# PJLab-ADG/OpenPCSeg

Measured on AMD Instinct MI355X. Metric: LiDAR frames/sec training MinkUNet-34 SemanticKITTI, higher is better.
Workload: dtype f32; 1 GPU; MinkUNet-34 cr1.0 train step, 12 x 120k-pt synthetic SemanticKITTI scans/GPU, fp32; global_batch=12, voxels_per_gpu_batch=1158864, parallelism=dp1, wgrad=fp32

## Files before the change

include/pcseg_hip.h:

```cpp
#ifndef PCSEG_HIP_H_
#define PCSEG_HIP_H_

#include <stddef.h>
#include <stdint.h>

#ifdef __cplusplus
extern "C" {
#endif

#define PCS_OK 0
#define PCS_EINVAL (-1)
#define PCS_EWORKSPACE (-2)
#define PCS_ELAUNCH (-3)
#define PCS_EUNSUPPORTED (-4)

#define PCS_ABI_VERSION 12

int pcs_abi_version(void);
const char *pcs_last_error(void);

int pcs_hash(const int32_t *coords, int64_t n, int64_t *out, void *stream);

int pcs_kernel_hash(const int32_t *coords, int64_t n, const int32_t *offsets, int32_t K,
                    int64_t *out, void *stream);
// ... 128 lines not shown
                             void *stream);
int pcs_range_sample_bwd_csr_f32(const float *gout, const int64_t *order, const int64_t *rowptr, const float *wts,
                                 int32_t B, int32_t C, int32_t H, int32_t W, float *gimg, void *stream);

int32_t pcs_bn_num_partials(void);
int pcs_bn_stats_f32(const float *x, int64_t n, int32_t c, float *partial_ws, double *sums, void *stream);
int pcs_bn_reduce_partials(const double *partial, int64_t nrows, int32_t c, int64_t n, double *sums, void *stream);
int pcs_bn_reduce_partials_finalize(const double *partial, int64_t nrows, int32_t c, int64_t n, double eps, double momentum,
                                    float *running_mean, float *running_var, double *sums, double *stat, void *stream);
int pcs_bn_finalize_f32(const double *sums, double count, const double *count_dev, int32_t c, double eps,
                        double momentum, float *running_mean, float *running_var, double *stat, void *stream);
int pcs_bn_apply_f32(const float *x, const float *res, const double *stat, const float *w, const float *b,
                     int64_t n, int32_t c, int32_t relu, float *y, uint32_t *mask, int64_t ldy, const float *tail,
                     int32_t ctail, void *stream);
int pcs_bn_bwd_stats_f32(const float *dy, const float *x, const float *y, const uint32_t *mask, const double *stat,
                         int64_t n, int32_t c, int32_t relu, float *partial_ws, double *sums2, int64_t sums2_doubles,
                         int64_t lddy, void *stream);
int pcs_bn_bwd_apply_f32(const float *dy, const float *x, const float *y, const uint32_t *mask, const double *stat,
                         const double *sums2, double count, const double *count_dev, const float *w, int64_t n,
                         int32_t c, int32_t relu, float *dx, float *dres, int64_t lddy, void *stream);
int pcs_bn_stats_h(const void *x, int64_t n, int32_t c, int32_t dtype, float *partial_ws, double *sums, void *stream);
int pcs_bn_apply_h(const void *x, const void *res, const double *stat, const float *w, const float *b, int64_t n,
                   int32_t c, int32_t relu, int32_t dtype, void *y, uint32_t *mask, int64_t ldy, const void *tail,
                   int32_t ctail, void *stream);
int pcs_bn_bwd_stats_h(const void *dy, const void *x, const void *y, const uint32_t *mask, const double *stat, int64_t n,
                       int32_t c, int32_t relu, int32_t dtype, float *partial_ws, double *sums2, int64_t sums2_doubles,
                       int64_t lddy, void *stream);
int pcs_bn_bwd_apply_h(const void *dy, const void *x, const void *y, const uint32_t *mask, const double *stat,
                       const double *sums2, double count, const double *count_dev, const float *w, int64_t n,
                       int32_t c, int32_t relu, int32_t dtype, void *dx, void *dres, int64_t lddy, void *stream);
int pcs_bn_bwd_apply_act(const void *dy, const void *x, const void *y, const uint32_t *mask, const double *stat,
                         const double *sums2, double count, const double *count_dev, const float *w, int64_t n, int32_t c,
                         int32_t relu, int32_t dtype, float in_slope, void *dx, void *dres, int64_t lddy, void *stream);

int pcs_recon_gate_f32(const float *a0, const float *a1, const float *a2, const float *x, const double *stat3,
                       const float *gamma3, const float *beta3, int64_t n, int32_t c, float *out, void *stream);
int pcs_recon_gate_h(const void *a0, const void *a1, const void *a2, const void *x, const double *stat3, const float *gamma3,
                     const float *beta3, int64_t n, int32_t c, int32_t dtype, void *out, void *stream);
int pcs_recon_gate_bwd_stats_f32(const float *dy, const float *x, const float *a0, const float *a1, const float *a2,
                                 const double *stat3, const float *gamma3, const float *beta3, int64_t n, int32_t c,
                                 float *partial_ws, double *sums2, int64_t sums2_doubles, void *stream);
int pcs_recon_gate_bwd_stats_h(const void *dy, const void *x, const void *a0, const void *a1, const void *a2,
                               const double *stat3, const float *gamma3, const float *beta3, int64_t n, int32_t c,
                               int32_t dtype, float *partial_ws, double *sums2, int64_t sums2_doubles, void *stream);
int pcs_recon_gate_bwd_apply_f32(const float *dy, const float *x, const float *a0, const float *a1, const float *a2,
                                 const double *stat3, const float *gamma3, const float *beta3, const double *sums2,
                                 double count, const double *count_dev, int64_t n, int32_t c, float *dx_gate, float *da0,
                                 float *da1, float *da2, void *stream);
int pcs_recon_gate_bwd_apply_h(const void *dy, const void *x, const void *a0, const void *a1, const void *a2,
                               const double *stat3, const float *gamma3, const float *beta3, const double *sums2, double count,
                               const double *count_dev, int64_t n, int32_t c, int32_t dtype, void *dx_gate, void *da0,
                               void *da1, void *da2, void *stream);

int pcs_quantize_floor(const void *points, int32_t is_float, int64_t n, int32_t row_stride,
                       const double *voxel_size3, int32_t *coords, int32_t *bbox, void *stream);
int pcs_quantize_keys(const int32_t *coords, int64_t n, const int32_t *bbox, int64_t *keys, void *stream);
int pcs_quantize_frame_keys(const int32_t *coords, const int64_t *frames, int64_t n, const int32_t *bbox, int64_t *keys, void *stream);
int pcs_quantize_flags(const int64_t *sorted_keys, int64_t n, int32_t *flags, void *stream);
int pcs_quantize_emit(const int32_t *flags, const int64_t *rank, const int64_t *perm, const int32_t *coords,
                      int64_t n, int32_t *vox, int64_t *index, int64_t *inverse, void *stream);

int pcs_unique_emit(const int32_t *flags, const int64_t *rank, const int64_t *perm, const int64_t *sorted_keys,
                    int64_t n, int64_t *uniq, int64_t *inverse, int64_t *rowptr, void *stream);

int pcs_conv_x3_applies(int32_t cin, int32_t cout, int32_t K);
int32_t pcs_conv_x3_column_tiles(int32_t cout);
// ... 65 lines not shown
```

openpcseg_amd/csrc/norm.hip:

```cpp
#include "row_storage.h"

using namespace pcs;

namespace {

template <int V> struct NV;
template <> struct NV<4> { using T = float4; };
template <> struct NV<1> { using T = float; };
template <int V, typename ET> __device__ __forceinline__ typename NV<V>::T ldv(ET, const void *p, int64_t e) {
  const Acc<V> a = widen(ET{}, *reinterpret_cast<const typename Raw<ET, V>::T *>(reinterpret_cast<const typename Elem<ET>::T *>(p) + e));
  if constexpr (V == 4) return make_float4(a.f[0], a.f[1], a.f[2], a.f[3]);
  else return a.f[0];
}
template <typename ET> __device__ __forceinline__ void stv(ET, void *p, int64_t e, const float4 &v) {
  *reinterpret_cast<typename Raw<ET, 4>::T *>(reinterpret_cast<typename Elem<ET>::T *>(p) + e) = narrow(ET{}, Acc<4>{{v.x, v.y, v.z, v.w}});
}
template <typename ET> __device__ __forceinline__ void stv(ET, void *p, int64_t e, const float &v) {
  reinterpret_cast<typename Elem<ET>::T *>(p)[e] = narrow(ET{}, Acc<1>{{v}});
}

__device__ __forceinline__ float comp(const float4 &v, int i) { return i == 0 ? v.x : (i == 1 ? v.y : (i == 2 ? v.z : v.w)); }
__device__ __forceinline__ float comp(const float &v, int) { return v; }
__device__ __forceinline__ void setc(float4 &v, int i, float s) { if (i == 0) v.x = s; else if (i == 1) v.y = s; else if (i == 2) v.z = s; else v.w = s; }
__device__ __forceinline__ void setc(float &v, int, float s) { v = s; }
// ... 211 lines not shown
  if (!(count > 0.0)) count = 1.0;
  for (int j = threadIdx.x; j < cv; j += blockDim.x) {
    float mean[V], invstd[V], k1[V], k2[V], ws[V];
#pragma unroll
    for (int q = 0; q < V; ++q) {
      const int ch = j * V + q;
      mean[q] = (float)stat[ch]; invstd[q] = (float)stat[c + ch];
      k1[q] = (float)(sums2[ch] / count);
      k2[q] = (float)(sums2[c + ch] / count);
      ws[q] = invstd[q] * (w ? w[ch] : 1.f);
    }
#pragma unroll 4
    for (int64_t i = (int64_t)blockIdx.x * blockDim.y + threadIdx.y; i < n; i += (int64_t)gridDim.x * blockDim.y) {
      const VT gv = ldv<V>(ET{}, dy, i * lddy + (int64_t)j * V);
      const VT xv = ldv<V>(ET{}, x, i * c + (int64_t)j * V);
      VT yv; unsigned bits = 0xFu;
      if (relu) {
        if (V == 4 && mask) bits = (mask[i * (c >> 5) + (j >> 3)] >> (4 * (j & 7))) & 0xFu;
        else yv = ldv<V>(ET{}, y, i * c + (int64_t)j * V);
      }
      VT o, r;
#pragma unroll
      for (int q = 0; q < V; ++q) {
        float g = comp(gv, q);
        if (relu && ((V == 4 && mask) ? !((bits >> q) & 1u) : comp(yv, q) <= 0.f)) g = 0.f;
        const float xh = (comp(xv, q) - mean[q]) * invstd[q];
        float d = (g - k1[q] - xh * k2[q]) * ws[q];
        if (in_slope != 1.f && !(comp(xv, q) > 0.f)) d *= in_slope;
        setc(o, q, d);
        setc(r, q, g);
      }
      stv(ET{}, dx, i * c + (int64_t)j * V, o);
      if (dres) stv(ET{}, dres, i * c + (int64_t)j * V, r);
    }
  }
}

template <int V> RowLaunch geo(int64_t n, int c) { return row_launch(n, c / V, kRowsExact4); }

}

extern "C" int32_t pcs_bn_num_partials(void) { return kStatBlocks + 1; }

static bool al_v4(int dtype, const void *p) { return aligned(p, dtype == 0 ? 16 : 8); }

static int bn_partial(bool bwd, int dtype, const void *x, const void *dy, const void *y, const uint32_t *mask, const double *stat,
                      int64_t n, int c, int relu, float *partial, double *sums, hipStream_t st, int64_t lddy = 0) {
  if (lddy == 0) lddy = c;
  if (lddy < c) { set_error("pcs_bn: row stride of dy smaller than c"); return PCS_EINVAL; }
  const bool vec = (c & 3) == 0 && (lddy & 3) == 0 && al_v4(dtype, x) && al_v4(dtype, dy) && al_v4(dtype, y);
  if (mask && (!vec || (c & 31))) { set_error("pcs_bn: the ReLU bit mask needs c % 32 == 0 and aligned rows"); return PCS_EUNSUPPORTED; }
  const int V = vec ? 4 : 1, cv = c / V;
  const dim3 block = row_launch(n, cv, kRowsExact4).block;
  const size_t lds = (size_t)block.y * 2 * block.x * V * sizeof(float);
  if (vec) {
    if (bwd) PCS_DTYPE(dtype, hipLaunchKernelGGL((bn_partial_kernel<true, 4, ET>), dim3(kStatBlocks), block, lds, st, x, dy, y, mask, stat, n, c, cv, relu, partial, lddy));
    else PCS_DTYPE(dtype, hipLaunchKernelGGL((bn_partial_kernel<false, 4, ET>), dim3(kStatBlocks), block, lds, st, x, dy, y, mask, stat, n, c, cv, relu, partial, lddy));
  } else {
    if (bwd) PCS_DTYPE(dtype, hipLaunchKernelGGL((bn_partial_kernel<true, 1, ET>), dim3(kStatBlocks), block, lds, st, x, dy, y, mask, stat, n, c, cv, relu, partial, lddy));
    else PCS_DTYPE(dtype, hipLaunchKernelGGL((bn_partial_kernel<false, 1, ET>), dim3(kStatBlocks), block, lds, st, x, dy, y, mask, stat, n, c, cv, relu, partial, lddy));
  }
  const float *pivot = bwd ? nullptr : partial + (size_t)kStatBlocks * 2 * c;
  hipLaunchKernelGGL(bn_reduce_kernel<float>, dim3((unsigned)ceil_div(c, kRedCh)), dim3(kRedCh, kRedLanes), 0, st, partial, kStatBlocks, c,
                     pivot, n, sums, bwd ? 0 : 1, bwd ? reinterpret_cast<float *>(sums + 2 * (size_t)c) : (float *)nullptr,
                     (double *)nullptr, 0.0, 0.0, (float *)nullptr, (float *)nullptr);
  return check_launch("pcs_bn_partial");
// ... 99 lines not shown
                                    double *sums2, int64_t sums2_doubles, int64_t lddy, void *stream) {
  if (n < 0 || c <= 0 || (n > 0 && (!dy || !x || (relu && !y && !mask))) || !stat || !partial_ws || !sums2) { set_error("pcs_bn_bwd_stats: bad args"); return PCS_EINVAL; }
  if (sums2_doubles < 3 * (int64_t)c) { set_error("pcs_bn_bwd_stats: sums2 must hold 3c doubles (2c sums + the same 2c values as floats)"); return PCS_EWORKSPACE; }
  return bn_partial(true, 0, x, dy, y, mask, stat, n, c, relu, partial_ws, sums2, as_stream(stream), lddy);
}
extern "C" int pcs_bn_bwd_stats_h(const void *dy, const void *x, const void *y, const uint32_t *mask,
                                  const double *stat, int64_t n, int32_t c, int32_t relu, int32_t dtype, float *partial_ws,
                                  double *sums2, int64_t sums2_doubles, int64_t lddy, void *stream) {
  if (n < 0 || c <= 0 || (n > 0 && (!dy || !x || (relu && !y && !mask))) || !stat || !partial_ws || !sums2 || !is_half(dtype)) { set_error("pcs_bn_bwd_stats_h: bad args"); return PCS_EINVAL; }
  if (sums2_doubles < 3 * (int64_t)c) { set_error("pcs_bn_bwd_stats_h: sums2 must hold 3c doubles (2c sums + the same 2c values as floats)"); return PCS_EWORKSPACE; }
  return bn_partial(true, dtype, x, dy, y, mask, stat, n, c, relu, partial_ws, sums2, as_stream(stream), lddy);
}

extern "C" int pcs_bn_bwd_apply_f32(const float *dy, const float *x, const float *y, const uint32_t *mask,
                                    const double *stat, const double *sums2, double count, const double *count_dev,
                                    const float *w, int64_t n, int32_t c, int32_t relu, float *dx, float *dres,
                                    int64_t lddy, void *stream) {
  return bn_bwd_apply_any(0, dy, x, y, mask, stat, sums2, count, count_dev, w, n, c, relu, dx, dres, lddy, stream);
}
extern "C" int pcs_bn_bwd_apply_act(const void *dy, const void *x, const void *y, const uint32_t *mask,
                                    const double *stat, const double *sums2, double count, const double *count_dev,
                                    const float *w, int64_t n, int32_t c, int32_t relu, int32_t dtype, float in_slope, void *dx,
                                    void *dres, int64_t lddy, void *stream) {
  if (dtype < 0 || dtype > 2 || !(in_slope > 0.f)) { set_error("pcs_bn_bwd_apply_act: dtype must be 0 / 1 / 2 and in_slope > 0"); return PCS_EINVAL; }
  return bn_bwd_apply_any(dtype, dy, x, y, mask, stat, sums2, count, count_dev, w, n, c, relu, dx, dres, lddy, stream, in_slope);
}
extern "C" int pcs_bn_bwd_apply_h(const void *dy, const void *x, const void *y, const uint32_t *mask,
                                  const double *stat, const double *sums2, double count, const double *count_dev,
                                  const float *w, int64_t n, int32_t c, int32_t relu, int32_t dtype, void *dx, void *dres,
                                  int64_t lddy, void *stream) {
  if (bad_half("pcs_bn_bwd_apply_h", dtype, false)) return PCS_EINVAL;
  return bn_bwd_apply_any(dtype, dy, x, y, mask, stat, sums2, count, count_dev, w, n, c, relu, dx, dres, lddy, stream);
}
```

openpcseg_amd/fused.py:

```python
import torch
import torch.distributed as dist
from torch import nn
from torch.autograd import Function

from . import native
from .sparse import SparseTensor


def _world():
    return dist.get_world_size() if dist.is_available() and dist.is_initialized() else 1


def _syncing(sync):
    if not sync or not (dist.is_available() and dist.is_initialized()):
        return False
    import os
    return dist.get_world_size() > 1 or os.environ.get("PCS_SYNC_WORLD1") == "1"


_STATS_GROUP = {}


def _stats_group():
    import os
# ... 66 lines not shown
        ctx.in_slope = in_slope
        return y

    @staticmethod
    def backward(ctx, dy):
        be = native.backend()
        x, gate, stat, weight, count_dev = ctx.saved_tensors
        count, relu, sync, has_res, has_tail = ctx.cfg
        c = x.shape[1]
        dtail = None
        if has_tail:
            dtail = dy[:, c:]
            dy = dy[:, :c]
        else:
            dy = dy.contiguous()
        local = be.bn_bwd_stats(dy, x, gate, stat, relu)
        sums2 = local
        if _syncing(sync):
            sums2 = local.clone()
            dist.all_reduce(sums2, group=_stats_group())
        if ctx.in_slope is not None:
            dx, dres = be.bn_bwd_apply(dy, x, gate, stat, sums2, count, weight, relu, has_res, count_dev=count_dev, in_slope=ctx.in_slope)
        else:
            dx, dres = be.bn_bwd_apply(dy, x, gate, stat, sums2, count, weight, relu, has_res, count_dev=count_dev)
        dw = db = None
        if weight is not None:
            lw = getattr(local, "_pcs_f32", None)
            if lw is None or lw.dtype != weight.dtype:
                lw = local.to(weight.dtype)
            dw, db = lw[c:], lw[:c]
        return dx, dres, dw, db, None, None, None, None, None, None, None, None, None, dtail, None


class FusedBatchNorm(nn.Module):

    def __init__(self, num_features, eps=1e-5, momentum=0.1, sync=False):
        super().__init__()
        self.num_features, self.eps, self.momentum, self.sync = num_features, eps, momentum, sync
        self.weight = nn.Parameter(torch.ones(num_features))
        self.bias = nn.Parameter(torch.zeros(num_features))
        self.register_buffer("running_mean", torch.zeros(num_features))
        self.register_buffer("running_var", torch.ones(num_features))
        self.register_buffer("num_batches_tracked", torch.tensor(0, dtype=torch.long))
        self.counted_by_parent = False

    def extra_repr(self):
        return "%d, eps=%g, momentum=%g, sync=%s" % (self.num_features, self.eps, self.momentum, self.sync)

    def forward(self, input, residual=None, relu=False, cat_with=None, in_slope=None):
        x = input.feats
        r = residual.feats if isinstance(residual, SparseTensor) else residual
        tail = cat_with.feats if isinstance(cat_with, SparseTensor) else cat_with
        if tail is not None and (x.shape[1] % 4 or tail.shape[1] % 4 or tail.shape[0] != x.shape[0]):
            y = self.forward(input, residual=residual, relu=relu)
            return input._like(torch.cat([y.feats, tail.to(y.feats.dtype)], dim=1))
        if self.training:
            if not self.counted_by_parent:
                self.num_batches_tracked += 1
            pre = getattr(input, "bn_sums", None)
            if pre is not None:
                sums, of, ver = pre
                pre = sums if (of is x and x._version == ver) else None
            y = _FusedBN.apply(x, r, self.weight, self.bias, self.running_mean, self.running_var, self.eps,
                               self.momentum, relu, self.sync, input.cmaps, input.stride, pre, tail, in_slope)
        else:
            inv = torch.rsqrt(self.running_var.double() + self.eps)
            stat = torch.cat([self.running_mean.double(), inv]).contiguous()
            y = native.backend().bn_apply(x.contiguous(), r.contiguous() if r is not None else None, stat,
                                          self.weight, self.bias, relu, tail=tail.contiguous() if tail is not None else None)
        return input._like(y)


class _SkinnyLinear(Function):

    @staticmethod
    def forward(ctx, x, weight, bias, cache, hd=None):
        from . import functional as F_
        be = native.backend()
        km = F_._identity_map(x.shape[0], x.device, cache)
        w1 = weight.detach().float().t().contiguous().unsqueeze(0)
        fam = F_._conv_family(be, hd, x.is_cuda, w1.shape[1], w1.shape[2], 1, x3=False)
        y, x, _ = F_._run_conv(be, fam, x, w1, km, hd, F_._per_call, bias=bias.float() if bias is not None else None)
# ... 433 lines not shown
```

openpcseg_amd/native.py:

```python
import ctypes
import os
from ctypes import c_char_p, c_double, c_float, c_int32, c_int64, c_size_t, c_void_p

import torch

_LIB_PATH = os.environ.get("PCS_LIB_PATH") or os.path.join(os.path.dirname(os.path.abspath(__file__)), "lib",
                                                          "libpcseg_hip.so")

_P = c_void_p
SIGNATURES = {
    "pcs_abi_version": (c_int32, []),
    "pcs_last_error": (c_char_p, []),
    "pcs_hash": (c_int32, [_P, c_int64, _P, _P]),
    "pcs_kernel_hash": (c_int32, [_P, c_int64, _P, c_int32, _P, _P]),
    "pcs_hashtable_capacity": (c_int64, [c_int64]),
    "pcs_hashtable_bytes": (c_size_t, [c_int64]),
    "pcs_hashtable_build": (c_int32, [_P, c_int64, _P, c_int64, _P]),
    "pcs_hashtable_query": (c_int32, [_P, c_int64, _P, c_int64, _P, _P]),
    "pcs_count": (c_int32, [_P, c_int64, _P, c_int64, _P]),
    "pcs_voxelize_fwd_f32": (c_int32, [_P, _P, _P, c_int64, c_int64, c_int32, _P, _P]),
    "pcs_voxelize_fwd_csr_f32": (c_int32, [_P, _P, _P, _P, c_int64, c_int32, _P, _P]),
    "pcs_voxelize_bwd_f32": (c_int32, [_P, _P, _P, c_int64, c_int32, _P, _P]),
    "pcs_devoxelize_fwd_f32": (c_int32, [_P, _P, _P, c_int64, c_int32, _P, _P]),
    "pcs_devoxelize_bwd_f32": (c_int32, [_P, _P, _P, c_int64, c_int64, c_int32, _P, _P]),
# ... 39 lines not shown
    "pcs_conv_gather_gemm_f32_ex": (c_int32, [_P, c_int64, c_int32, _P, c_int32, c_int32, _P, c_int32,
                                              _P, c_int32, c_int64, _P, _P, _P, _P, _P, _P]),
    "pcs_conv_supports_epilogue": (c_int32, [c_int32, c_int32, c_int32, c_int32]),
    "pcs_bn_bwd_apply_act": (c_int32, [_P, _P, _P, _P, _P, _P, c_double, _P, _P, c_int64, c_int32, c_int32, c_int32, c_float, _P, _P,
                                       c_int64, _P]),
    "pcs_bn_reduce_partials": (c_int32, [_P, c_int64, c_int32, c_int64, _P, _P]),
    "pcs_bn_reduce_partials_finalize": (c_int32, [_P, c_int64, c_int32, c_int64, c_double, c_double, _P, _P, _P, _P, _P]),
    "pcs_transpose_kab_f32": (c_int32, [_P, c_int32, c_int32, c_int32, _P, _P]),
    "pcs_conv_wgrad_ws_bytes": (c_size_t, [_P, c_int32, c_int32, c_int32]),
    "pcs_conv_wgrad_f32": (c_int32, [_P, c_int32, _P, c_int32, _P, c_int32, _P, _P, c_int32, _P,
                                     _P, c_size_t, _P]),
    "pcs_scatter_max_fwd_f32": (c_int32, [_P, _P, _P, c_int64, c_int32, _P, _P, _P]),
    "pcs_scatter_max_bwd_f32": (c_int32, [_P, _P, c_int64, c_int64, c_int32, _P, _P]),
    "pcs_map_count": (c_int32, [_P, c_int64, c_int32, c_int32, c_int32, _P, _P]),
    "pcs_denselize_fwd_f32": (c_int32, [_P, _P, _P, c_int64, c_int32, c_int32, c_int32, c_int32, _P, _P]),
    "pcs_denselize_fwd_csr_f32": (c_int32, [_P, _P, _P, _P, c_int32, c_int32, c_int32, c_int32, _P, _P]),
    "pcs_denselize_bwd_csr_f32": (c_int32, [_P, _P, _P, _P, c_int64, c_int32, c_int32, c_int32, c_int32, _P, _P]),
    "pcs_denselize_bwd_f32": (c_int32, [_P, _P, _P, c_int64, c_int32, c_int32, c_int32, c_int32, _P, _P]),
    "pcs_range_sample_fwd_f32": (c_int32, [_P, _P, c_int64, c_int32, c_int32, c_int32, c_int32, _P, _P]),
    "pcs_range_sample_corners": (c_int32, [_P, c_int64, c_int32, c_int32, c_int32, _P, _P, _P]),
    "pcs_range_sample_bwd_csr_f32": (c_int32, [_P, _P, _P, _P, c_int32, c_int32, c_int32, c_int32, _P, _P]),
    "pcs_bn_num_partials": (c_int32, []),
    "pcs_bn_stats_f32": (c_int32, [_P, c_int64, c_int32, _P, _P, _P]),
    "pcs_bn_finalize_f32": (c_int32, [_P, c_double, _P, c_int32, c_double, c_double, _P, _P, _P, _P]),
    "pcs_bn_apply_f32": (c_int32, [_P, _P, _P, _P, _P, c_int64, c_int32, c_int32, _P, _P, c_int64, _P, c_int32, _P]),
    "pcs_bn_bwd_stats_f32": (c_int32, [_P, _P, _P, _P, _P, c_int64, c_int32, c_int32, _P, _P, c_int64, c_int64, _P]),
    "pcs_bn_bwd_apply_f32": (c_int32, [_P, _P, _P, _P, _P, _P, c_double, _P, _P, c_int64, c_int32, c_int32, _P, _P,
                                       c_int64, _P]),
    "pcs_bn_stats_h": (c_int32, [_P, c_int64, c_int32, c_int32, _P, _P, _P]),
    "pcs_bn_apply_h": (c_int32, [_P, _P, _P, _P, _P, c_int64, c_int32, c_int32, c_int32, _P, _P, c_int64, _P, c_int32, _P]),
    "pcs_bn_bwd_stats_h": (c_int32, [_P, _P, _P, _P, _P, c_int64, c_int32, c_int32, c_int32, _P, _P, c_int64, c_int64, _P]),
    "pcs_bn_bwd_apply_h": (c_int32, [_P, _P, _P, _P, _P, _P, c_double, _P, _P, c_int64, c_int32, c_int32, c_int32, _P, _P,
                                     c_int64, _P]),
    "pcs_quantize_floor": (c_int32, [_P, c_int32, c_int64, c_int32, _P, _P, _P, _P]),
    "pcs_quantize_keys": (c_int32, [_P, c_int64, _P, _P, _P]),
    "pcs_quantize_frame_keys": (c_int32, [_P, _P, c_int64, _P, _P, _P]),
    "pcs_quantize_flags": (c_int32, [_P, c_int64, _P, _P]),
    "pcs_quantize_emit": (c_int32, [_P, _P, _P, _P, c_int64, _P, _P, _P, _P]),
    "pcs_conv_h_applies": (c_int32, [c_int32, c_int32, c_int32]),
    "pcs_conv_prepared_weights_bytes": (c_size_t, [c_int32, c_int32, c_int32]),
    "pcs_conv_prepare_weights_h": (c_int32, [_P, c_int32, c_int32, c_int32, c_int32, c_int32, _P, _P]),
    "pcs_conv_gather_gemm_h": (c_int32, [_P, c_int64, c_int32, _P, c_int32, c_int32, _P, c_int32, _P, c_int32, c_int64,
                                         _P, _P, c_int32, _P, _P, _P]),
    "pcs_conv_gather_gemm_h_ex": (c_int32, [_P, c_int64, c_int32, _P, c_int32, c_int32, _P, c_int32, _P, c_int32, c_int64,
                                            _P, _P, _P, c_int32, _P, _P, _P]),
    "pcs_conv_x3_applies": (c_int32, [c_int32, c_int32, c_int32]),
    "pcs_conv_x3_column_tiles": (c_int32, [c_int32]),
    "pcs_conv_x3_emits_bn_partials": (c_int32, [c_int32, c_int32, c_int32, c_int32]),
    "pcs_conv_prepared_weights_x3_bytes": (c_size_t, [c_int32, c_int32, c_int32]),
    "pcs_conv_prepare_weights_x3": (c_int32, [_P, c_int32, c_int32, c_int32, c_int32, _P, _P]),
    "pcs_conv_gather_gemm_f32_bf16x3": (c_int32, [_P, c_int64, c_int32, _P, c_int32, c_int32, _P, c_int32, _P, c_int32, c_int64,
                                                  _P, _P, _P, _P, _P]),
    "pcs_conv_wgrad_f32_bf16x3": (c_int32, [_P, c_int32, _P, c_int32, _P, c_int32, _P, _P, c_int32, _P,
                                            _P, c_size_t, _P]),
    "pcs_conv_wgrad_h": (c_int32, [_P, c_int32, _P, c_int32, _P, c_int32, _P, _P, c_int32, _P, _P, c_size_t, c_int32, _P]),
    "pcs_unique_emit": (c_int32, [_P, _P, _P, _P, c_int64, _P, _P, _P, _P]),
    "pcs_cylinder_partition_f32": (c_int32, [_P, c_int64, c_int32, _P, _P, _P, _P, _P, _P, _P]),
    "pcs_voxel_label_vote": (c_int32, [_P, _P, c_int64, c_int64, c_int32, c_int64, _P, _P, _P, _P]),
    "pcs_rows_argmax_gather_f32": (c_int32, [_P, c_int64, c_int32, _P, c_int64, _P, _P]),
    "pcs_predict_points_f32": (c_int32, [_P, c_int64, c_int32, _P, c_int64, _P, _P, c_int32, _P, _P, _P, _P, _P, _P]),
    "pcs_weights_multi_plan": (c_int64, [_P, c_int32]),
    "pcs_weights_multi": (c_int32, [_P, c_int32, c_int64, _P]),
    "pcs_lovasz_workspace_bytes": (c_int64, [c_int64, c_int32, c_int32, c_int64]),
    "pcs_lovasz_softmax_f32": (c_int32, [_P, _P, c_int64, c_int32, c_int32, c_int64, _P, _P, _P, c_int64, _P]),
    "pcs_debug_convh_ws": (None, [c_int32, c_int32, c_int32]),
    "pcs_debug_wgrad_interleave": (None, [c_int32]),
# ... 847 lines not shown
        if not ok:
            t = t.contiguous()
        return t, t.stride(0)

    def bn_bwd_stats(self, dy, x, gate, stat, relu):
        x = self._feat(x, "input")
        n, c = x.shape
        dy, lddy = self._rows(dy, "grad_output", x, c)
        ws = torch.empty(self.lib.pcs_bn_num_partials() * 2 * c, dtype=torch.float32, device=x.device)
        buf = torch.empty(3 * c, dtype=torch.float64, device=x.device)
        sums2 = buf[:2 * c]
        sums2._pcs_f32 = buf[2 * c:].view(torch.float32)
        yp, mp = self._gate(gate, relu)
        self._twin("pcs_bn_bwd_stats", self._CODE[x.dtype], [_ptr(dy), _ptr(x), yp, mp, _ptr(stat), n, c, int(relu)],
                   [_ptr(ws), _ptr(sums2), buf.numel(), lddy, _stream()])
        return sums2

    def bn_bwd_apply(self, dy, x, gate, stat, sums2, count, w, relu, want_res, count_dev=None, in_slope=None):
        x = self._feat(x, "input")
        n, c = x.shape
        dy, lddy = self._rows(dy, "grad_output", x, c)
        dx = torch.empty_like(x)
        dres = torch.empty_like(x) if want_res else None
        yp, mp = self._gate(gate, relu)
        if in_slope is not None and float(in_slope) != 1.0:
            _check(self.lib.pcs_bn_bwd_apply_act(_ptr(dy), _ptr(x), yp, mp, _ptr(stat), _ptr(sums2), float(count), _ptr(count_dev),
                                                 _ptr(w), n, c, int(relu), self._CODE[x.dtype], float(in_slope),
                                                 _ptr(dx), _ptr(dres), lddy, _stream()), "pcs_bn_bwd_apply_act")
            return dx, dres
        self._twin("pcs_bn_bwd_apply", self._CODE[x.dtype],
                   [_ptr(dy), _ptr(x), yp, mp, _ptr(stat), _ptr(sums2), float(count), _ptr(count_dev), _ptr(w), n, c, int(relu)],
                   [_ptr(dx), _ptr(dres), lddy, _stream()])
        return dx, dres

    def _recon_rows(self, tensors):
        ts = [self._feat(t, "input") for t in tensors]
        dt = ts[0].dtype if all(t.dtype == ts[0].dtype for t in ts) else torch.float32
        ts = [(t if t.dtype == dt else t.to(dt)).contiguous() for t in ts]
        if any(t.dim() != 2 or t.shape != ts[0].shape for t in ts):
            raise ValueError("openpcseg_amd: the recon gate takes (n, c) tensors of one shape, got %s" % [tuple(t.shape) for t in ts])
        return ts, self._CODE[dt]

    def recon_gate(self, a3, x, stat3, gamma3, beta3):
        (a0, a1, a2, x), code = self._recon_rows(list(a3) + [x])
        n, c = x.shape
        out = torch.empty_like(x)
        self._twin("pcs_recon_gate", code, [_ptr(a0), _ptr(a1), _ptr(a2), _ptr(x), _ptr(stat3), _ptr(gamma3), _ptr(beta3), n, c],
                   [_ptr(out), _stream()])
        return out

    def recon_gate_bwd_stats(self, dy, x, a3, stat3, gamma3, beta3):
        (dy, x, a0, a1, a2), code = self._recon_rows([dy, x] + list(a3))
        n, c = x.shape
        buf = torch.empty(9 * c, dtype=torch.float64, device=x.device) if n > 0 else \
            torch.zeros(9 * c, dtype=torch.float64, device=x.device)
        ws = torch.empty(self.lib.pcs_bn_num_partials() * 6 * c, dtype=torch.float32, device=x.device)
        sums2 = buf[:6 * c]
        sums2._pcs_f32 = buf[6 * c:].view(torch.float32)
        self._twin("pcs_recon_gate_bwd_stats", code,
                   [_ptr(dy), _ptr(x), _ptr(a0), _ptr(a1), _ptr(a2), _ptr(stat3), _ptr(gamma3), _ptr(beta3), n, c],
                   [_ptr(ws), _ptr(sums2), buf.numel(), _stream()])
        return sums2

    def recon_gate_bwd_apply(self, dy, x, a3, stat3, gamma3, beta3, sums2, count, count_dev=None):
        (dy, x, a0, a1, a2), code = self._recon_rows([dy, x] + list(a3))
        n, c = x.shape
# ... 198 lines not shown
```

openpcseg_amd/workloads/minkunet.py:

```python
import os

import torch
from torch import nn

from .. import functional as F
from .. import inference
from .. import modules as spnn
from ..fused import FusedBatchNorm, FusedLinear
from ..sparse import PointTensor, cat, fapply
from .losses import SegLoss
from .pointvoxel import initial_voxelize, point_maps, voxel_to_point

MK34_LAYERS = [2, 3, 4, 6, 2, 2, 2, 2]
MK18_LAYERS = [2, 2, 2, 2, 2, 2, 2, 2]
PLANES = [32, 32, 64, 128, 256, 256, 128, 96, 96]


class _BN(nn.BatchNorm1d):
    def forward(self, x):
        return fapply(x, super().forward)


class _SyncBN(nn.SyncBatchNorm):
    def forward(self, x):
        return fapply(x, super().forward)


FUSED = True


def _norm(c, dist):
    if FUSED:
        return FusedBatchNorm(c, sync=dist)
    return _SyncBN(c) if dist else _BN(c)


def _link(conv, bn):
    if isinstance(bn, FusedBatchNorm) and isinstance(conv, spnn.Conv3d):
        conv.emit_bn_stats = os.environ.get("PCS_CONV_BN_STATS", "1") != "0"


CAT_FUSED = os.environ.get("PCS_CAT_FUSED", "1") != "0"
PREBUILD = os.environ.get("PCS_PREBUILD_LEVELS", "1") != "0"
SKIP_FUSED = os.environ.get("PCS_SKIP_FUSED", "1") != "0"


def _bn_act(bn, x, residual=None, relu=True, act=None, cat_with=None):
    if isinstance(bn, FusedBatchNorm):
        if cat_with is not None and not CAT_FUSED:
            return cat([bn(x, residual=residual, relu=relu), cat_with])
        return bn(x, residual=residual, relu=relu, cat_with=cat_with)
    y = bn(x)
    if residual is not None:
        y = y + residual
    y = act(y) if relu else y
    return y if cat_with is None else cat([y, cat_with])


class ConvBlock(nn.Module):

    def __init__(self, cin, cout, ks, stride, dist, transposed=False):
        super().__init__()
        self.net = nn.Sequential(spnn.Conv3d(cin, cout, kernel_size=ks, stride=stride, transposed=transposed),
                                 _norm(cout, dist), spnn.ReLU(True))
        _link(self.net[0], self.net[1])

    def forward(self, x, cat_with=None):
        folds = inference.active(self)
        if folds is not None:
            y = folds["net"](x)
            return y if cat_with is None else cat([y, cat_with])
        return _bn_act(self.net[1], self.net[0](x), act=self.net[2], cat_with=cat_with)


class ResBlock(nn.Module):
    def __init__(self, cin, cout, dist):
        super().__init__()
        self.net = nn.Sequential(spnn.Conv3d(cin, cout, kernel_size=3), _norm(cout, dist), spnn.ReLU(True),
                                 spnn.Conv3d(cout, cout, kernel_size=3), _norm(cout, dist))
        if cin == cout:
            self.downsample = nn.Identity()
        else:
            self.downsample = nn.Sequential(spnn.Conv3d(cin, cout, kernel_size=1), _norm(cout, dist))
        self.relu = spnn.ReLU(True)
        _link(self.net[0], self.net[1])
        _link(self.net[3], self.net[4])

    def forward(self, x):
        folds = inference.active(self)
        if folds is not None:
            r = x if folds["ds"] is None else folds["ds"](x)
            return folds["b"](folds["a"](x), residual=r)
        if SKIP_FUSED and torch.is_grad_enabled() and x.feats.requires_grad:
            h0, xs = self.net[0](x, with_skip=True)
        else:
            h0, xs = self.net[0](x), x
        h = _bn_act(self.net[1], h0, act=self.net[2])
        if isinstance(self.downsample, nn.Identity):
            r = xs
        else:
            r = _bn_act(self.downsample[1], self.downsample[0](xs), relu=False)
        return _bn_act(self.net[4], self.net[3](h), residual=r, act=self.relu)


def _res_stack(cin, cout, n, dist):
    return [ResBlock(cin if i == 0 else cout, cout, dist) for i in range(n)]


class MinkUNet(nn.Module):
    point_branch = False

    def __init__(self, num_class=20, in_dim=4, num_layer=MK34_LAYERS, planes=PLANES, cr=1.0,
                 pres=0.05, vres=0.05, dist=False, ignore_label=0, label_smoothing=0.1, dropout=0.0):
        super().__init__()
        cs = [int(cr * c) for c in planes]
        self.in_dim, self.pres, self.vres = in_dim, pres, vres
        self.stem = nn.Sequential(spnn.Conv3d(in_dim, cs[0], kernel_size=3), _norm(cs[0], dist), spnn.ReLU(True),
                                  spnn.Conv3d(cs[0], cs[0], kernel_size=3), _norm(cs[0], dist), spnn.ReLU(True))
        _link(self.stem[0], self.stem[1])
        _link(self.stem[3], self.stem[4])
        enc_in = [cs[0], cs[1], cs[2], cs[3]]
        for i in range(4):
            setattr(self, "stage%d" % (i + 1), nn.Sequential(
                ConvBlock(enc_in[i], enc_in[i], 2, 2, dist), *_res_stack(enc_in[i], cs[i + 1], num_layer[i], dist)))
        skip = [cs[3], cs[2], cs[1], cs[0]]
        cin = cs[4]
        for i in range(4):
            cout = cs[5 + i]
            setattr(self, "up%d" % (i + 1), nn.ModuleList([
                ConvBlock(cin, cout, 2, 2, dist, transposed=True),
                nn.Sequential(*_res_stack(cout + skip[i], cout, num_layer[4 + i], dist))]))
            cin = cout
# ... 81 lines not shown
```

Baseline: 106.3 frames/s.

## Fuse main-branch and shortcut BatchNorm apply and backward into dual kernels

Residual blocks with a projection shortcut now normalize both the main conv output and the downsample conv output in one kernel that also adds, applies ReLU and writes the mask. The backward pass computes both branches' gradient statistics and input gradients in one shared pass over dy. This removes the intermediate shortcut BN output tensor and one extra read/write pass over the activations in both directions. It only covers the few downsampling blocks and adds new code paths that must match the single-BN numerics.

Result: no change. 107.1 frames/s, median of 6 (+0.7%).

```diff
diff --git a/include/pcseg_hip.h b/include/pcseg_hip.h
--- a/include/pcseg_hip.h
+++ b/include/pcseg_hip.h
@@ -184,6 +184,24 @@
 int pcs_bn_bwd_apply_act(const void *dy, const void *x, const void *y, const uint32_t *mask, const double *stat,
                          const double *sums2, double count, const double *count_dev, const float *w, int64_t n, int32_t c,
                          int32_t relu, int32_t dtype, float in_slope, void *dx, void *dres, int64_t lddy, void *stream);
+int pcs_bn_apply2_f32(const float *xa, const float *xb, const double *stat_a, const double *stat_b, const float *wa,
+                      const float *ba, const float *wb, const float *bb, int64_t n, int32_t c, float *y, uint32_t *mask,
+                      void *stream);
+int pcs_bn_apply2_h(const void *xa, const void *xb, const double *stat_a, const double *stat_b, const float *wa,
+                    const float *ba, const float *wb, const float *bb, int64_t n, int32_t c, int32_t dtype, void *y,
+                    uint32_t *mask, void *stream);
+int pcs_bn_bwd_stats2_f32(const float *dy, const float *xa, const float *xb, const uint32_t *mask, const double *stat_a,
+                          const double *stat_b, int64_t n, int32_t c, float *partial_ws, double *sums2, int64_t sums2_doubles,
+                          void *stream);
+int pcs_bn_bwd_stats2_h(const void *dy, const void *xa, const void *xb, const uint32_t *mask, const double *stat_a,
+                        const double *stat_b, int64_t n, int32_t c, int32_t dtype, float *partial_ws, double *sums2,
+                        int64_t sums2_doubles, void *stream);
+int pcs_bn_bwd_apply2_f32(const float *dy, const float *xa, const float *xb, const uint32_t *mask, const double *stat_a,
+                          const double *stat_b, const double *sums2, double count, const double *count_dev, const float *wa,
+                          const float *wb, int64_t n, int32_t c, float *dxa, float *dxb, void *stream);
+int pcs_bn_bwd_apply2_h(const void *dy, const void *xa, const void *xb, const uint32_t *mask, const double *stat_a,
+                        const double *stat_b, const double *sums2, double count, const double *count_dev, const float *wa,
+                        const float *wb, int64_t n, int32_t c, int32_t dtype, void *dxa, void *dxb, void *stream);
 
 int pcs_recon_gate_f32(const float *a0, const float *a1, const float *a2, const float *x, const double *stat3,
                        const float *gamma3, const float *beta3, int64_t n, int32_t c, float *out, void *stream);
diff --git a/openpcseg_amd/csrc/norm.hip b/openpcseg_amd/csrc/norm.hip
--- a/openpcseg_amd/csrc/norm.hip
+++ b/openpcseg_amd/csrc/norm.hip
@@ -267,6 +267,158 @@
       }
       stv(ET{}, dx, i * c + (int64_t)j * V, o);
       if (dres) stv(ET{}, dres, i * c + (int64_t)j * V, r);
+    }
+  }
+}
+
+
+template <int V, typename ET>
+__global__ void __launch_bounds__(256) bn_apply2_kernel(const void *__restrict__ xa, const void *__restrict__ xb,
+                                                        const double *__restrict__ stata, const double *__restrict__ statb,
+                                                        const float *__restrict__ wa, const float *__restrict__ ba,
+                                                        const float *__restrict__ wb, const float *__restrict__ bb, int64_t n,
+                                                        int c, int cv, void *__restrict__ y, uint32_t *__restrict__ mask) {
+#pragma clang fp contract(off)
+  using VT = typename NV<V>::T;
+  for (int j = threadIdx.x; j < cv; j += blockDim.x) {
+    float sca[V], sha[V], scb[V], shb[V];
+#pragma unroll
+    for (int q = 0; q < V; ++q) {
+      const int ch = j * V + q;
+      const float invstda = (float)stata[c + ch], meana = (float)stata[ch];
+      sca[q] = invstda * (wa ? wa[ch] : 1.f);
+      sha[q] = fmaf(-meana, sca[q], ba ? ba[ch] : 0.f);
+      const float invstdb = (float)statb[c + ch], meanb = (float)statb[ch];
+      scb[q] = invstdb * (wb ? wb[ch] : 1.f);
+      shb[q] = fmaf(-meanb, scb[q], bb ? bb[ch] : 0.f);
+    }
+#pragma unroll 4
+    for (int64_t i = (int64_t)blockIdx.x * blockDim.y + threadIdx.y; i < n; i += (int64_t)gridDim.x * blockDim.y) {
+      const VT xav = ldv<V>(ET{}, xa, i * c + (int64_t)j * V);
+      const VT xbv = ldv<V>(ET{}, xb, i * c + (int64_t)j * V);
+      VT o;
+      unsigned bits = 0;
+#pragma unroll
+      for (int q = 0; q < V; ++q) {
+        const float r = stored(ET{}, fmaf(comp(xbv, q), scb[q], shb[q]));
+        float t = fmaf(comp(xav, q), sca[q], sha[q]);
+        t += r;
+        if (t < 0.f) t = 0.f;
+        setc(o, q, t);
+        bits |= (stored(ET{}, t) > 0.f ? 1u : 0u) << q;
+      }
+      stv(ET{}, y, i * c + (int64_t)j * V, o);
+      unsigned m = bits << (4 * (j & 7));
+      m |= __shfl_xor(m, 1, 64); m |= __shfl_xor(m, 2, 64); m |= __shfl_xor(m, 4, 64);
+      if ((j & 7) == 0) mask[i * (c >> 5) + (j >> 3)] = m;
+    }
+  }
+}
+
+template <int V, typename ET>
+__global__ void __launch_bounds__(256) bn_partial2_kernel(const void *__restrict__ xa, const void *__restrict__ xb,
+                                                          const void *__restrict__ dy, const uint32_t *__restrict__ mask,
+                                                          const double *__restrict__ stata, const double *__restrict__ statb,
+                                                          int64_t n, int c, int cv, float *__restrict__ partial) {
+#pragma clang fp contract(off)
+  using VT = typename NV<V>::T;
+  extern __shared__ float red[];
+  const int tx = threadIdx.x, ty = threadIdx.y, TX = blockDim.x, TY = blockDim.y;
+  const int W = TX * V;
+  for (int j0 = 0; j0 < cv; j0 += TX) {
+    const int j = j0 + tx;
+    float s0[V], s1a[V], s1b[V];
+#pragma unroll
+    for (int q = 0; q < V; ++q) { s0[q] = 0.f; s1a[q] = 0.f; s1b[q] = 0.f; }
+    if (j < cv) {
+      float meana[V], invstda[V], meanb[V], invstdb[V];
+#pragma unroll
+      for (int q = 0; q < V; ++q) {
+        meana[q] = (float)stata[j * V + q]; invstda[q] = (float)stata[c + j * V + q];
+        meanb[q] = (float)statb[j * V + q]; invstdb[q] = (float)statb[c + j * V + q];
+      }
+#pragma unroll 4
+      for (int64_t i = (int64_t)blockIdx.x * TY + ty; i < n; i += (int64_t)gridDim.x * TY) {
+        const VT xav = ldv<V>(ET{}, xa, i * c + (int64_t)j * V);
+        const VT xbv = ldv<V>(ET{}, xb, i * c + (int64_t)j * V);
+        const VT gv = ldv<V>(ET{}, dy, i * c + (int64_t)j * V);
+        const unsigned bits = (mask[i * (c >> 5) + (j >> 3)] >> (4 * (j & 7))) & 0xFu;
+#pragma unroll
+        for (int q = 0; q < V; ++q) {
+          float g = comp(gv, q);
+          if (!((bits >> q) & 1u)) g = 0.f;
+          s0[q] += g;
+          s1a[q] = fmaf(g, (comp(xav, q) - meana[q]) * invstda[q], s1a[q]);
+          s1b[q] = fmaf(g, (comp(xbv, q) - meanb[q]) * invstdb[q], s1b[q]);
+        }
+      }
+    }
+#pragma unroll
+    for (int q = 0; q < V; ++q) {
+      red[(ty * 3 + 0) * W + tx * V + q] = s0[q];
+      red[(ty * 3 + 1) * W + tx * V + q] = s1a[q];
+      red[(ty * 3 + 2) * W + tx * V + q] = s1b[q];
+    }
+    __syncthreads();
+    if (ty == 0 && j < cv) {
+#pragma unroll
+      for (int q = 0; q < V; ++q) {
+        float a = 0.f, b = 0.f, d = 0.f;
+        for (int r = 0; r < TY; ++r) {
+          a += red[(r * 3 + 0) * W + tx * V + q]; b += red[(r * 3 + 1) * W + tx * V + q]; d += red[(r * 3 + 2) * W + tx * V + q];
+        }
+        float *row = partial + (int64_t)blockIdx.x * 4 * c + j * V + q;
+        row[0] = a; row[c] = b; row[2 * c] = a; row[3 * c] = d;
+      }
+    }
+    __syncthreads();
+  }
+}
+
+template <int V, typename ET>
+__global__ void __launch_bounds__(256) bn_bwd_apply2_kernel(const void *__restrict__ dy, const void *__restrict__ xa,
+                                                            const void *__restrict__ xb, const uint32_t *__restrict__ mask,
+                                                            const double *__restrict__ stata, const double *__restrict__ statb,
+                                                            const double *__restrict__ sums2, double count,
+                                                            const double *__restrict__ count_dev, const float *__restrict__ wa,
+                                                            const float *__restrict__ wb, int64_t n, int c, int cv,
+                                                            void *__restrict__ dxa, void *__restrict__ dxb) {
+#pragma clang fp contract(off)
+  using VT = typename NV<V>::T;
+  if (count_dev) count = *count_dev;
+  if (!(count > 0.0)) count = 1.0;
+  for (int j = threadIdx.x; j < cv; j += blockDim.x) {
+    float meana[V], invstda[V], k1a[V], k2a[V], wsa[V], meanb[V], invstdb[V], k1b[V], k2b[V], wsb[V];
+#pragma unroll
+    for (int q = 0; q < V; ++q) {
+      const int ch = j * V + q;
+      meana[q] = (float)stata[ch]; invstda[q] = (float)stata[c + ch];
+      k1a[q] = (float)(sums2[ch] / count);
+      k2a[q] = (float)(sums2[c + ch] / count);
+      wsa[q] = invstda[q] * (wa ? wa[ch] : 1.f);
+      meanb[q] = (float)statb[ch]; invstdb[q] = (float)statb[c + ch];
+      k1b[q] = (float)(sums2[2 * c + ch] / count);
+      k2b[q] = (float)(sums2[3 * c + ch] / count);
+      wsb[q] = invstdb[q] * (wb ? wb[ch] : 1.f);
+    }
+#pragma unroll 4
+    for (int64_t i = (int64_t)blockIdx.x * blockDim.y + threadIdx.y; i < n; i += (int64_t)gridDim.x * blockDim.y) {
+      const VT gv = ldv<V>(ET{}, dy, i * c + (int64_t)j * V);
+      const VT xav = ldv<V>(ET{}, xa, i * c + (int64_t)j * V);
+      const VT xbv = ldv<V>(ET{}, xb, i * c + (int64_t)j * V);
+      const unsigned bits = (mask[i * (c >> 5) + (j >> 3)] >> (4 * (j & 7))) & 0xFu;
+      VT oa, ob;
+#pragma unroll
+      for (int q = 0; q < V; ++q) {
+        float g = comp(gv, q);
+        if (!((bits >> q) & 1u)) g = 0.f;
+        const float xha = (comp(xav, q) - meana[q]) * invstda[q];
+        setc(oa, q, fmaf(-xha, k2a[q], g - k1a[q]) * wsa[q]);
+        const float xhb = (comp(xbv, q) - meanb[q]) * invstdb[q];
+        setc(ob, q, fmaf(-xhb, k2b[q], g - k1b[q]) * wsb[q]);
+      }
+      stv(ET{}, dxa, i * c + (int64_t)j * V, oa);
+      stv(ET{}, dxb, i * c + (int64_t)j * V, ob);
     }
   }
 }
@@ -432,3 +584,92 @@
   if (bad_half("pcs_bn_bwd_apply_h", dtype, false)) return PCS_EINVAL;
   return bn_bwd_apply_any(dtype, dy, x, y, mask, stat, sums2, count, count_dev, w, n, c, relu, dx, dres, lddy, stream);
 }
+
+static bool dual_serves(const char *what, int dtype, int32_t c, std::initializer_list<const void *> rows) {
+  bool ok = (c & 31) == 0;
+  for (const void *p : rows) ok = ok && al_v4(dtype, p);
+  if (!ok) set_error("%s: the dual pass needs c %% 32 == 0 and aligned rows", what);
+  return ok;
+}
+
+static int bn_apply2_any(int dtype, const void *xa, const void *xb, const double *stat_a, const double *stat_b, const float *wa,
+                         const float *ba, const float *wb, const float *bb, int64_t n, int32_t c, void *y, uint32_t *mask,
+                         void *stream) {
+  if (n < 0 || c <= 0) { set_error("pcs_bn_apply2: bad sizes"); return PCS_EINVAL; }
+  if (n == 0) return PCS_OK;
+  if (!xa || !xb || !stat_a || !stat_b || !y || !mask) { set_error("pcs_bn_apply2: null pointer"); return PCS_EINVAL; }
+  if (!dual_serves("pcs_bn_apply2", dtype, c, {xa, xb, y})) return PCS_EUNSUPPORTED;
+  const RowLaunch g = geo<4>(n, c);
+  PCS_DTYPE(dtype, hipLaunchKernelGGL((bn_apply2_kernel<4, ET>), g.grid, g.block, 0, as_stream(stream), xa, xb, stat_a, stat_b, wa, ba,
+                                      wb, bb, n, c, g.cv, y, mask));
+  return check_launch("pcs_bn_apply2");
+}
+
+static int bn_bwd_stats2_any(int dtype, const void *dy, const void *xa, const void *xb, const uint32_t *mask, const double *stat_a,
+                             const double *stat_b, int64_t n, int32_t c, float *partial_ws, double *sums2, int64_t sums2_doubles,
+                             void *stream) {
+  if (n < 0 || c <= 0 || (n > 0 && (!dy || !xa || !xb || !mask)) || !stat_a || !stat_b || !partial_ws || !sums2) {
+    set_error("pcs_bn_bwd_stats2: bad args");
+    return PCS_EINVAL;
+  }
+  if (sums2_doubles < 6 * (int64_t)c) { set_error("pcs_bn_bwd_stats2: sums2 must hold 6c doubles (4c sums + the same 4c values as floats)"); return PCS_EWORKSPACE; }
+  if (!dual_serves("pcs_bn_bwd_stats2", dtype, c, {dy, xa, xb})) return PCS_EUNSUPPORTED;
+  hipStream_t st = as_stream(stream);
+  const int cv = c / 4;
+  const dim3 block = row_launch(n, cv, kRowsExact4).block;
+  const size_t lds = (size_t)block.y * 3 * block.x * 4 * sizeof(float);
+  PCS_DTYPE(dtype, hipLaunchKernelGGL((bn_partial2_kernel<4, ET>), dim3(kStatBlocks), block, lds, st, xa, xb, dy, mask, stat_a, stat_b, n, c, cv, partial_ws));
+  hipLaunchKernelGGL(bn_reduce_kernel<float>, dim3((unsigned)ceil_div(2 * c, kRedCh)), dim3(kRedCh, kRedLanes), 0, st, partial_ws, kStatBlocks,
+                     2 * c, (const float *)nullptr, n, sums2, 0, reinterpret_cast<float *>(sums2 + 4 * (size_t)c), (double *)nullptr, 0.0,
+                     0.0, (float *)nullptr, (float *)nullptr);
+  return check_launch("pcs_bn_bwd_stats2");
+}
+
+static int bn_bwd_apply2_any(int dtype, const void *dy, const void *xa, const void *xb, const uint32_t *mask, const double *stat_a,
+                             const double *stat_b, const double *sums2, double count, const double *count_dev, const float *wa,
+                             const float *wb, int64_t n, int32_t c, void *dxa, void *dxb, void *stream) {
+  if (n < 0 || c <= 0) { set_error("pcs_bn_bwd_apply2: bad sizes"); return PCS_EINVAL; }
+  if (n == 0) return PCS_OK;
+  if (!count_dev && !(count > 0)) { set_error("pcs_bn_bwd_apply2: count must be positive"); return PCS_EINVAL; }
+  if (!dy || !xa || !xb || !mask || !stat_a || !stat_b || !sums2 || !dxa || !dxb) { set_error("pcs_bn_bwd_apply2: null pointer"); return PCS_EINVAL; }
+  if (!dual_serves("pcs_bn_bwd_apply2", dtype, c, {dy, xa, xb, dxa, dxb})) return PCS_EUNSUPPORTED;
+  const RowLaunch g = geo<4>(n, c);
+  PCS_DTYPE(dtype, hipLaunchKernelGGL((bn_bwd_apply2_kernel<4, ET>), g.grid, g.block, 0, as_stream(stream), dy, xa, xb, mask, stat_a, stat_b,
+                                      sums2, count, count_dev, wa, wb, n, c, g.cv, dxa, dxb));
+  return check_launch("pcs_bn_bwd_apply2");
+}
+
+extern "C" int pcs_bn_apply2_f32(const float *xa, const float *xb, const double *stat_a, const double *stat_b, const float *wa,
+                                 const float *ba, const float *wb, const float *bb, int64_t n, int32_t c, float *y, uint32_t *mask,
+                                 void *stream) {
+  return bn_apply2_any(0, xa, xb, stat_a, stat_b, wa, ba, wb, bb, n, c, y, mask, stream);
+}
+extern "C" int pcs_bn_apply2_h(const void *xa, const void *xb, const double *stat_a, const double *stat_b, const float *wa,
+                               const float *ba, const float *wb, const float *bb, int64_t n, int32_t c, int32_t dtype, void *y,
+                               uint32_t *mask, void *stream) {
+  if (bad_half("pcs_bn_apply2_h", dtype)) return PCS_EINVAL;
+  return bn_apply2_any(dtype, xa, xb, stat_a, stat_b, wa, ba, wb, bb, n, c, y, mask, stream);
+}
+extern "C" int pcs_bn_bwd_stats2_f32(const float *dy, const float *xa, const float *xb, const uint32_t *mask, const double *stat_a,
+                                     const double *stat_b, int64_t n, int32_t c, float *partial_ws, double *sums2,
+                                     int64_t sums2_doubles, void *stream) {
+  return bn_bwd_stats2_any(0, dy, xa, xb, mask, stat_a, stat_b, n, c, partial_ws, sums2, sums2_doubles, stream);
+}
+extern "C" int pcs_bn_bwd_stats2_h(const void *dy, const void *xa, const void *xb, const uint32_t *mask, const double *stat_a,
+                                   const double *stat_b, int64_t n, int32_t c, int32_t dtype, float *partial_ws, double *sums2,
+                                   int64_t sums2_doubles, void *stream) {
+  if (bad_half("pcs_bn_bwd_stats2_h", dtype)) return PCS_EINVAL;
+  return bn_bwd_stats2_any(dtype, dy, xa, xb, mask, stat_a, stat_b, n, c, partial_ws, sums2, sums2_doubles, stream);
+}
+extern "C" int pcs_bn_bwd_apply2_f32(const float *dy, const float *xa, const float *xb, const uint32_t *mask, const double *stat_a,
+                                     const double *stat_b, const double *sums2, double count, const double *count_dev,
+                                     const float *wa, const float *wb, int64_t n, int32_t c, float *dxa, float *dxb, void *stream) {
+  return bn_bwd_apply2_any(0, dy, xa, xb, mask, stat_a, stat_b, sums2, count, count_dev, wa, wb, n, c, dxa, dxb, stream);
+}
+extern "C" int pcs_bn_bwd_apply2_h(const void *dy, const void *xa, const void *xb, const uint32_t *mask, const double *stat_a,
+                                   const double *stat_b, const double *sums2, double count, const double *count_dev,
+                                   const float *wa, const float *wb, int64_t n, int32_t c, int32_t dtype, void *dxa, void *dxb,
+                                   void *stream) {
+  if (bad_half("pcs_bn_bwd_apply2_h", dtype)) return PCS_EINVAL;
+  return bn_bwd_apply2_any(dtype, dy, xa, xb, mask, stat_a, stat_b, sums2, count, count_dev, wa, wb, n, c, dxa, dxb, stream);
+}
diff --git a/openpcseg_amd/fused.py b/openpcseg_amd/fused.py
--- a/openpcseg_amd/fused.py
+++ b/openpcseg_amd/fused.py
@@ -122,6 +122,46 @@
         return dx, dres, dw, db, None, None, None, None, None, None, None, None, None, dtail, None
 
 
+class _FusedBN2(Function):
+
+    @staticmethod
+    def forward(ctx, xa, xb, wa, ba, wb, bb, bn_a, bn_b, pre_a, pre_b):
+        be = native.backend()
+        xa, xb = xa.contiguous(), xb.contiguous()
+        stat_b, _, _ = _train_stat(be, xb, pre_b, bn_b.sync, bn_b.eps, bn_b.momentum, bn_b.running_mean, bn_b.running_var)
+        stat_a, count, count_dev = _train_stat(be, xa, pre_a, bn_a.sync, bn_a.eps, bn_a.momentum, bn_a.running_mean, bn_a.running_var)
+        y, mask = be.bn_apply2(xa, xb, stat_a, stat_b, wa, ba, wb, bb)
+        ctx.save_for_backward(xa, xb, mask, stat_a, stat_b, wa, wb, count_dev)
+        ctx.cfg = (count, bn_a.sync)
+        return y
+
+    @staticmethod
+    def backward(ctx, dy):
+        be = native.backend()
+        xa, xb, mask, stat_a, stat_b, wa, wb, count_dev = ctx.saved_tensors
+        count, sync = ctx.cfg
+        c = xa.shape[1]
+        dy = dy.contiguous()
+        if dy.data_ptr() % (4 * dy.element_size()):
+            dy = dy.clone()
+        local = be.bn_bwd_stats2(dy, xa, xb, mask, stat_a, stat_b)
+        sums2 = local
+        if _syncing(sync):
+            sums2 = local.clone()
+            dist.all_reduce(sums2, group=_stats_group())
+        dxa, dxb = be.bn_bwd_apply2(dy, xa, xb, mask, stat_a, stat_b, sums2, count, wa, wb, count_dev=count_dev)
+        lw = getattr(local, "_pcs_f32", None)
+        if lw is None or lw.dtype != wa.dtype:
+            lw = local.to(wa.dtype)
+        return dxa, dxb, lw[c:2 * c], lw[:c], lw[3 * c:], lw[2 * c:3 * c], None, None, None, None
+
+
+def _dual_enabled(be, bn_a, bn_b, xa, xb, relu):
+    return (relu and isinstance(bn_a, FusedBatchNorm) and isinstance(bn_b, FusedBatchNorm) and bn_a.training and bn_b.training and
+            bn_a.sync == bn_b.sync and hasattr(be, "bn_apply2") and isinstance(xa, torch.Tensor) and isinstance(xb, torch.Tensor) and
+            bn_a.weight.dtype == bn_b.weight.dtype and be.bn_dual_serves(xa.contiguous(), xb.contiguous()))
+
+
 class FusedBatchNorm(nn.Module):
 
     def __init__(self, num_features, eps=1e-5, momentum=0.1, sync=False):
@@ -137,7 +177,20 @@
     def extra_repr(self):
         return "%d, eps=%g, momentum=%g, sync=%s" % (self.num_features, self.eps, self.momentum, self.sync)
 
-    def forward(self, input, residual=None, relu=False, cat_with=None, in_slope=None):
+    def forward(self, input, residual=None, relu=False, cat_with=None, in_slope=None, residual_bn=None):
+        if residual_bn is not None:
+            bn_r, r_in = residual_bn
+            if residual is None and cat_with is None and in_slope is None and isinstance(r_in, SparseTensor):
+                xa, pre_a = _feats_pre(input)
+                xb, pre_b = _feats_pre(r_in)
+                if _dual_enabled(native.backend(), self, bn_r, xa, xb, relu):
+                    for bn in (self, bn_r):
+                        if not bn.counted_by_parent:
+                            bn.num_batches_tracked += 1
+                    return input._like(_FusedBN2.apply(xa, xb, self.weight, self.bias, bn_r.weight, bn_r.bias, self, bn_r,
+                                                       pre_a, pre_b))
+            assert residual is None, "residual and residual_bn are two spellings of the one residual"
+            residual = bn_r(r_in)
         x = input.feats
         r = residual.feats if isinstance(residual, SparseTensor) else residual
         tail = cat_with.feats if isinstance(cat_with, SparseTensor) else cat_with
diff --git a/openpcseg_amd/native.py b/openpcseg_amd/native.py
--- a/openpcseg_amd/native.py
+++ b/openpcseg_amd/native.py
@@ -95,6 +95,12 @@
     "pcs_bn_bwd_stats_h": (c_int32, [_P, _P, _P, _P, _P, c_int64, c_int32, c_int32, c_int32, _P, _P, c_int64, c_int64, _P]),
     "pcs_bn_bwd_apply_h": (c_int32, [_P, _P, _P, _P, _P, _P, c_double, _P, _P, c_int64, c_int32, c_int32, c_int32, _P, _P,
                                      c_int64, _P]),
+    "pcs_bn_apply2_f32": (c_int32, [_P] * 8 + [c_int64, c_int32, _P, _P, _P]),
+    "pcs_bn_apply2_h": (c_int32, [_P] * 8 + [c_int64, c_int32, c_int32, _P, _P, _P]),
+    "pcs_bn_bwd_stats2_f32": (c_int32, [_P] * 6 + [c_int64, c_int32, _P, _P, c_int64, _P]),
+    "pcs_bn_bwd_stats2_h": (c_int32, [_P] * 6 + [c_int64, c_int32, c_int32, _P, _P, c_int64, _P]),
+    "pcs_bn_bwd_apply2_f32": (c_int32, [_P] * 7 + [c_double, _P, _P, _P, c_int64, c_int32, _P, _P, _P]),
+    "pcs_bn_bwd_apply2_h": (c_int32, [_P] * 7 + [c_double, _P, _P, _P, c_int64, c_int32, c_int32, _P, _P, _P]),
     "pcs_quantize_floor": (c_int32, [_P, c_int32, c_int64, c_int32, _P, _P, _P, _P]),
     "pcs_quantize_keys": (c_int32, [_P, c_int64, _P, _P, _P]),
     "pcs_quantize_frame_keys": (c_int32, [_P, _P, c_int64, _P, _P, _P]),
@@ -1008,6 +1014,51 @@
                    [_ptr(dy), _ptr(x), yp, mp, _ptr(stat), _ptr(sums2), float(count), _ptr(count_dev), _ptr(w), n, c, int(relu)],
                    [_ptr(dx), _ptr(dres), lddy, _stream()])
         return dx, dres
+
+    @staticmethod
+    def bn_dual_serves(*rows):
+        x = rows[0]
+        return (all(isinstance(t, torch.Tensor) and t.is_cuda and t.dim() == 2 and t.shape == x.shape and t.dtype == x.dtype
+                    for t in rows) and x.dtype in HipBackend._CODE and x.shape[1] % 32 == 0 and
+                all(t.is_contiguous() and t.data_ptr() % (4 * t.element_size()) == 0 for t in rows))
+
+    def bn_apply2(self, xa, xb, stat_a, stat_b, wa, ba, wb, bb):
+        xa = self._feat(xa, "input")
+        xb = self._feat(xb, "shortcut input", xa)
+        n, c = xa.shape
+        if xb.shape != xa.shape or c % 32:
+            raise RuntimeError("openpcseg_amd: the dual BatchNorm pass needs two (n, c) tensors of one shape with c a multiple of 32")
+        y = torch.empty_like(xa)
+        mask = torch.empty((n, c // 32), dtype=torch.int32, device=xa.device)
+        self._twin("pcs_bn_apply2", self._CODE[xa.dtype],
+                   [_ptr(xa), _ptr(xb), _ptr(stat_a), _ptr(stat_b), _ptr(wa), _ptr(ba), _ptr(wb), _ptr(bb), n, c],
+                   [_ptr(y), _ptr(mask), _stream()])
+        return y, mask
+
+    def bn_bwd_stats2(self, dy, xa, xb, mask, stat_a, stat_b):
+        xa = self._feat(xa, "input")
+        xb = self._feat(xb, "shortcut input", xa)
+        dy = self._feat(dy, "grad_output", xa)
+        n, c = xa.shape
+        ws = torch.empty(self.lib.pcs_bn_num_partials() * 4 * c, dtype=torch.float32, device=xa.device)
+        buf = torch.empty(6 * c, dtype=torch.float64, device=xa.device)
+        sums2 = buf[:4 * c]
+        sums2._pcs_f32 = buf[4 * c:].view(torch.float32)
+        self._twin("pcs_bn_bwd_stats2", self._CODE[xa.dtype],
+                   [_ptr(dy), _ptr(xa), _ptr(xb), _ptr(mask), _ptr(stat_a), _ptr(stat_b), n, c],
+                   [_ptr(ws), _ptr(sums2), buf.numel(), _stream()])
+        return sums2
+
+    def bn_bwd_apply2(self, dy, xa, xb, mask, stat_a, stat_b, sums2, count, wa, wb, count_dev=None):
+        xa = self._feat(xa, "input")
+        xb = self._feat(xb, "shortcut input", xa)
+        dy = self._feat(dy, "grad_output", xa)
+        n, c = xa.shape
+        dxa, dxb = torch.empty_like(xa), torch.empty_like(xb)
+        self._twin("pcs_bn_bwd_apply2", self._CODE[xa.dtype],
+                   [_ptr(dy), _ptr(xa), _ptr(xb), _ptr(mask), _ptr(stat_a), _ptr(stat_b), _ptr(sums2), float(count), _ptr(count_dev),
+                    _ptr(wa), _ptr(wb), n, c], [_ptr(dxa), _ptr(dxb), _stream()])
+        return dxa, dxb
 
     def _recon_rows(self, tensors):
         ts = [self._feat(t, "input") for t in tensors]
diff --git a/openpcseg_amd/workloads/minkunet.py b/openpcseg_amd/workloads/minkunet.py
--- a/openpcseg_amd/workloads/minkunet.py
+++ b/openpcseg_amd/workloads/minkunet.py
@@ -43,6 +43,7 @@
 CAT_FUSED = os.environ.get("PCS_CAT_FUSED", "1") != "0"
 PREBUILD = os.environ.get("PCS_PREBUILD_LEVELS", "1") != "0"
 SKIP_FUSED = os.environ.get("PCS_SKIP_FUSED", "1") != "0"
+DUAL_BN = os.environ.get("PCS_DUAL_BN", "1") != "0"
 
 
 def _bn_act(bn, x, residual=None, relu=True, act=None, cat_with=None):
@@ -98,6 +99,9 @@
         h = _bn_act(self.net[1], h0, act=self.net[2])
         if isinstance(self.downsample, nn.Identity):
             r = xs
+        elif DUAL_BN and isinstance(self.net[4], FusedBatchNorm) and isinstance(self.downsample[1], FusedBatchNorm):
+            xd = self.downsample[0](xs)
+            return self.net[4](self.net[3](h), relu=True, residual_bn=(self.downsample[1], xd))
         else:
             r = _bn_act(self.downsample[1], self.downsample[0](xs), relu=False)
         return _bn_act(self.net[4], self.net[3](h), residual=r, act=self.relu)
```
